# nubot-nudt/RDMNet

Hardware: AMD Instinct MI355X
Metric: scan-pairs/sec (whole node) (higher is better)
Workload: dtype f32

## Files before the change

### include/rdmnet_hip.h

```cpp
#ifndef RDMNET_HIP_H_
#define RDMNET_HIP_H_

#include <stddef.h>
#include <stdint.h>

#ifdef __cplusplus
extern "C" {
#endif

#define RDM_ABI_VERSION 2

int rdm_abi_version(void);
size_t rdm_abi_struct_size(int which);
const char* rdm_last_error(void);

int rdm_rehash_schedule(int64_t max_elems, int64_t* at_host, int64_t* buckets_host, int cap);

size_t rdm_grid_subsample_workspace_bytes(int64_t n_points, int batch);
int rdm_grid_subsample(const float* points, int64_t n_points, const int64_t* lengths, int batch,
                       float voxel_size, float* out_points, int64_t* out_lengths, void* ws,
                       size_t ws_bytes, void* stream);
int rdm_grid_subsample_form(const float* points, int64_t n_points, const int64_t* lengths, int batch, float voxel_size,
                            float* out_points, int64_t* out_lengths, void* ws, size_t ws_bytes, void* stream, int form);

// ... 47 lines not shown
                double* d2, double* totals_host, void* ws, size_t ws_bytes, void* stream);
int rdm_realign_error(const float* pts, int64_t n, int64_t ld, const double* gt_host, const double* est_host, double* mean_host,
                      void* ws, size_t ws_bytes, void* stream);

size_t rdm_information_workspace_bytes(int64_t n_q, int64_t n_s);
int rdm_information_matrix(const float* q, int64_t n_q, int64_t ld_q, const float* s, int64_t n_s, int64_t ld_s,
                           const double* q_transform_host, const double* s_transform_host, double cell, double radius,
                           double* out_host, int64_t* corr_out, int64_t capacity, void* ws, size_t ws_bytes, void* stream);

size_t rdm_gemm_workspace_bytes(int64_t m, int64_t n, int batches);
int rdm_gemm(const float* a, int64_t lda, int64_t stride_a, const float* b, int64_t ldb,
             int64_t stride_b, int trans_b, float* c, int64_t ldc, int64_t stride_c, int64_t m,
             int64_t n, int64_t k, int batches, const float* bias, const float* rowdiv, int act,
             void* ws, size_t ws_bytes, void* stream);
int rdm_gemm_last_plan(int* out4_host);

int rdm_kpconv_gather(const float* q_points, int64_t m, const float* s_points, int64_t n_s,
                      const float* s_feats, int64_t c, int64_t ldf, const uint8_t* s_positive,
                      const int64_t* idx, int64_t h, int64_t ldi, const int32_t* width,
                      const float* kernel_points, float sigma, float* wf, int64_t ldw, float* nn,
                      void* stream);
int rdm_kpconv_fused_enabled(void);
int rdm_kpconv_fused_supported(int64_t c_in, int64_t c_out);
int64_t rdm_kpconv_fused_partial_rows(int64_t m, int64_t c_in);
size_t rdm_kpconv_packed_floats(int64_t c_in, int64_t c_out);
int rdm_kpconv_pack_weights(const float* w_host, int64_t c_in, int64_t c_out, float* packed_host);
int rdm_kpconv_fused(const float* q_points, int64_t m, const float* s_points, int64_t n_s, const float* s_feats,
                     int64_t c, int64_t ldf, const uint8_t* s_positive, const int64_t* idx, int64_t h, int64_t ldi,
                     const int32_t* width, const float* kernel_points, float sigma, const float* w_packed,
                     const float* bias, int64_t c_out, float* out, int64_t ldo, double* gn_partial,
// ... 310 lines not shown
```

### rdmnet_amd/_lib.py

```python
import ctypes
import os

_HERE = os.path.dirname(os.path.abspath(__file__))
LIB_PATH = os.environ.get('RDM_LIB_PATH') or os.path.join(_HERE, 'librdmnet_hip.so')

c_void = ctypes.c_void_p
c_i64 = ctypes.c_int64
c_int = ctypes.c_int
c_f32 = ctypes.c_float
c_size = ctypes.c_size_t

ABI_VERSION = 2


class FineMatchingOptions(ctypes.Structure):
    _fields_ = [('topk', ctypes.c_int32), ('mutual', ctypes.c_int32), ('use_dustbin', ctypes.c_int32),
                ('use_global_score', ctypes.c_int32), ('confidence_threshold', ctypes.c_float),
                ('correspondence_limit', ctypes.c_int32)]

    @classmethod
    def of(cls, topk=1, mutual=False, use_dustbin=True, confidence_threshold=0.0, use_global_score=False,
           correspondence_limit=None):
        return cls(int(topk), int(bool(mutual)), int(bool(use_dustbin)), int(bool(use_global_score)), float(confidence_threshold),
                   0 if correspondence_limit is None else int(correspondence_limit))
# ... 28 lines not shown
    'rdm_grid_subsample': (c_int, [c_void, c_i64, c_void, c_int, c_f32, c_void, c_void, c_void, c_size,
                                   c_void]),
    'rdm_grid_subsample_form': (c_int, [c_void, c_i64, c_void, c_int, c_f32, c_void, c_void, c_void, c_size,
                                        c_void, c_int]),
    'rdm_radius_neighbors_workspace_bytes': (c_size, [c_i64, c_i64, c_int]),
    'rdm_radius_neighbors': (c_int, [c_void, c_i64, c_void, c_i64, c_void, c_void, c_int, c_f32, c_int,
                                     c_void, c_void, c_void, c_void, c_void, c_size, c_void]),
    'rdm_radius_grid_workspace_bytes': (c_size, [c_i64]),
    'rdm_radius_grid_build': (c_int, [c_void, c_i64, c_void, c_int, c_f32, c_void, c_size, c_void]),
    'rdm_radius_grid_query': (c_int, [c_void, c_size, c_i64, c_void, c_i64, c_void, c_int, c_f32, c_int, c_void, c_void,
                                      c_void, c_void, c_void, c_size, c_void]),
    'rdm_gemm_workspace_bytes': (c_size, [c_i64, c_i64, c_int]),
    'rdm_gemm': (c_int, [c_void, c_i64, c_i64, c_void, c_i64, c_i64, c_int, c_void, c_i64, c_i64, c_i64, c_i64,
                         c_i64, c_int, c_void, c_void, c_int, c_void, c_size, c_void]),
    'rdm_gemm_last_plan': (c_int, [c_void]),
    'rdm_kpconv_gather': (c_int, [c_void, c_i64, c_void, c_i64, c_void, c_i64, c_i64, c_void, c_void, c_i64,
                                  c_i64, c_void, c_void, c_f32, c_void, c_i64, c_void, c_void]),
    'rdm_kpconv_gather_ordered': (c_int, [c_void, c_i64, c_void, c_i64, c_void, c_i64, c_i64, c_void, c_void, c_i64,
                                          c_i64, c_void, c_void, c_f32, c_void, c_i64, c_void, c_void, c_void]),
    'rdm_kpconv_gather_form': (c_int, [c_void, c_i64, c_void, c_i64, c_void, c_i64, c_i64, c_void, c_void, c_i64,
                                       c_i64, c_void, c_void, c_f32, c_void, c_i64, c_void, c_void, c_int, c_void]),
    'rdm_kpconv_fused_enabled': (c_int, []),
    'rdm_kpconv_fused_supported': (c_int, [c_i64, c_i64]),
    'rdm_kpconv_fused_partial_rows': (c_i64, [c_i64, c_i64]),
    'rdm_kpconv_packed_floats': (c_size, [c_i64, c_i64]),
    'rdm_kpconv_pack_weights': (c_int, [c_void, c_i64, c_i64, c_void]),
    'rdm_kpconv_fused': (c_int, [c_void, c_i64, c_void, c_i64, c_void, c_i64, c_i64, c_void, c_void, c_i64, c_i64, c_void, c_void,
                                 c_f32, c_void, c_void, c_i64, c_void, c_i64, c_void, c_void, c_void]),
    'rdm_kpconv_fused_form': (c_int, [c_void, c_i64, c_void, c_i64, c_void, c_i64, c_i64, c_void, c_void, c_i64, c_i64, c_void, c_void,
                                      c_f32, c_void, c_void, c_i64, c_void, c_i64, c_void, c_void, c_int, c_void]),
# ... 195 lines not shown
```

### rdmnet_amd/csrc/engine.hip

```cpp
#include <algorithm>
#include <cmath>
#include <cstring>
#include <atomic>
#include <chrono>
#include <functional>
#include <map>
#include <memory>
#include <string>
#include <vector>

#include "../../include/rdmnet_hip.h"
#include <ctime>

#include "common.h"
#include "internal.h"
#include "lockstep.h"

namespace {

using namespace rdm;

struct Mat {
  float* p = nullptr;
  int64_t rows = 0, cols = 0, ld = 0;
// ... 944 lines not shown

extern "C" int rdm_engine_get_tensor(rdm_engine* e, const char* name, rdm_tensor_view* out) {
  RDM_REQUIRE(e && name && out, "rdm_engine_get_tensor: null pointer");
  auto it = e->taps.find(name);
  if (it == e->taps.end()) {
    set_error("rdm_engine_get_tensor: no tensor named %s (call rdm_engine_keep_taps first)", name);
    return RDM_ERR_ARG;
  }
  *out = it->second;
  return RDM_OK;
}

namespace {

struct PadGuard {
  explicit PadGuard(unsigned b) { rdm::gemm_set_lds_pad(b); }
  ~PadGuard() { rdm::gemm_set_lds_pad(0); }
};
struct CollateOnly {
  rdm_engine* e;
  bool keep_before;
  explicit CollateOnly(rdm_engine* eng) : e(eng), keep_before(eng->keep_taps) { e->keep_taps = e->collate_only = true; }
  ~CollateOnly() { e->collate_only = false; e->keep_taps = keep_before; }
};

int gs_multi_levels() {
  static const int n = [] { const char* v = ::rdm::dev_knob("RDM_GS_MULTI_LEVELS"); return v ? atoi(v) : 1; }();
  return n;
}

struct SearchQueue {
  std::vector<char> buf = std::vector<char>(radius_redo_queue_bytes());
// ... 76 lines not shown
static int grow_arena(rdm_engine* e, void* stream, const char* who) {
  RDM_HIP_CHECK(hipStreamSynchronize(static_cast<hipStream_t>(stream)));
  RDM_HIP_CHECK(hipFree(e->arena));
  e->arena = nullptr;
  e->arena_cap *= 2;
  const hipError_t err = hipMalloc(reinterpret_cast<void**>(&e->arena), e->arena_cap);
  if (err != hipSuccess) {
    e->arena_cap = 0;
    set_error("%s: growing the activation arena failed: %s", who, hipGetErrorString(err));
    return RDM_ERR_HIP;
  }
  return RDM_OK;
}
static int engine_run_growing(rdm_engine* e, const float* ref_points, int64_t n_ref, const float* src_points, int64_t n_src,
                              const rdm_data_dict* dd, rdm_engine_result* res, void* stream) {
  PadGuard pad_guard(e->pairs_in_flight >= 3 ? 20480u : 0u);
  for (;;) {
    e->arena_exhausted = false;
    const int rc = engine_run_once(e, ref_points, n_ref, src_points, n_src, dd, res, stream);
    if (!may_grow(e, rc)) return rc;
    ENG_CHECK(grow_arena(e, stream, "rdm_engine_run"));
  }
}

extern "C" int rdm_engine_run(rdm_engine* e, const float* ref_points, int64_t n_ref, const float* src_points,
                              int64_t n_src, rdm_engine_result* res, void* stream) {
  RDM_REQUIRE(e && ref_points && src_points && res, "rdm_engine_run: null pointer");
  RDM_REQUIRE(e->finalized, "rdm_engine_run: call rdm_engine_finalize first");
  RDM_REQUIRE(n_ref > 0 && n_src > 0, "rdm_engine_run: empty cloud");
  return engine_run_growing(e, ref_points, n_ref, src_points, n_src, nullptr, res, stream);
}
// ... 83 lines not shown
  for (;;) {
    e->arena_exhausted = false;
    const int rc = collate_batch_once(e, n_pairs, ref_points, n_ref, src_points, n_src, static_cast<hipStream_t>(stream));
    if (rc != RDM_OK) {
      e->batch.clear();
      e->arena_base = 0;
    }
    if (!may_grow(e, rc)) return rc;
    ENG_CHECK(grow_arena(e, stream, "rdm_engine_collate_batch"));
  }
}

extern "C" int rdm_engine_forward_batched(rdm_engine* e, int k, rdm_engine_result* res, void* stream) {
  RDM_REQUIRE(e && res, "rdm_engine_forward_batched: null pointer");
  RDM_REQUIRE(k >= 0 && k < static_cast<int>(e->batch.size()), "rdm_engine_forward_batched: no collated pair %d (rdm_engine_collate_batch first)", k);
  PadGuard pad_guard(e->pairs_in_flight >= 3 ? 20480u : 0u);
  e->arena_exhausted = false;
  return engine_run_once(e, nullptr, e->batch_n_ref[k], nullptr, e->batch_n_src[k], nullptr, res, stream, &e->batch[k]);
}

namespace {
int lockstep_wait(hipStream_t st, void* user) { return wait_idle(static_cast<rdm_engine*>(user), st); }

struct LockstepJob {
  const char* who;
  std::function<bool(int)> has_input;
  std::function<int(int)> check;
  std::function<int()> prepare;
  std::function<int(int)> pair;
  std::function<int(int)> rerun;
};

int lockstep_drive(const LockstepJob& job, rdm_engine* const* engines, rdm_engine_result* const* results, int n, void* stream) {
  const char* who = job.who;
  RDM_REQUIRE(n >= 1 && n <= kGroupMax, "%s: 1 .. %d pairs", who, kGroupMax);
  for (int k = 0; k < n; ++k) {
    RDM_REQUIRE(engines[k] && results[k] && job.has_input(k), "%s: pair %d is incomplete", who, k);
    RDM_REQUIRE(engines[k]->finalized, "%s: engine %d is not finalized", who, k);
    for (int j = 0; j < k; ++j) RDM_REQUIRE(engines[j] != engines[k], "%s: every pair needs an engine of its own", who);
    if (job.check) ENG_CHECK(job.check(k));
  }
  PadGuard pad_guard(0u);
  if (job.prepare) ENG_CHECK(job.prepare());
  struct Ctx {
    rdm_engine* const* engines;
    const LockstepJob* job;
  } ctx{engines, &job};
  auto run_pair = [](int k, void* user) -> int {
    const Ctx& c = *static_cast<const Ctx*>(user);
    c.engines[k]->arena_exhausted = false;
    return c.job->pair(k);
  };
  int rcs[kGroupMax] = {};
  const int wrc = lockstep_run(n, run_pair, &ctx, static_cast<hipStream_t>(stream), lockstep_wait, engines[0], rcs);
  if (wrc == -1) {
    set_error("%s: called from inside a lock-step group (a host thread runs one group at a time)", who);
    return RDM_ERR_ARG;
// ... 1096 lines not shown
```

### rdmnet_amd/csrc/gemm.hip

```cpp
#include "../../include/rdmnet_hip.h"
#include <cmath>
#include <cstdlib>

#include "common.h"
#include "internal.h"
#include "lockstep.h"

namespace {

using namespace rdm;

typedef float f32x16 __attribute__((ext_vector_type(16)));
typedef float f32x4_t __attribute__((ext_vector_type(4)));

struct GemmArgs {
  const float* A = nullptr;
  const float* B = nullptr;
  float* C = nullptr;
  const float* bias = nullptr;
  const float* rowdiv = nullptr;
  int M = 0, N = 0, K = 0;
  int lda = 0, ldb = 0, ldc = 0;
  long long sa = 0, sb = 0, sc = 0;
  int act = 0;
// ... 10 lines not shown
  unsigned long long* clk = nullptr;
#endif
};
#ifdef RDM_GEMM_TIMING
#define GEMM_STAMP(k) do { if (blockIdx.x == 0 && blockIdx.y == 0 && blockIdx.z == 0 && threadIdx.x == 0) g.clk[k] = __builtin_amdgcn_s_memtime(); } while (0)
#else
#define GEMM_STAMP(k) do { } while (0)
#endif

__device__ __forceinline__ float apply_act(float v, int act) {
  if (act == 1) return v > 0.f ? v : 0.f;
  if (act == 2) return v > 0.f ? v : 0.1f * v;
  return v;
}

template <int BM, int BN, int WM, int WN, int BK, bool TRANS_B, int PF, bool CAT = false>
__device__ __forceinline__ void gemm_kernel_body(const dim3 blockIdx, const dim3 gridDim, GemmArgs g) {
  (void)blockIdx; (void)gridDim;
  constexpr int TM = BM / WM, TN = BN / WN, FM = TM / 32, FN = TN / 32;
  static_assert(WM * WN == 4 && TM % 32 == 0 && TN % 32 == 0, "bad tile");
  constexpr int LDA_S = BM + 1, LDB_S = TRANS_B ? BN + 1 : BN + 4;
  constexpr int CR = BM < 64 ? BM : 64;
  constexpr int LDC_S = BN + 4;
  constexpr int TPR = BN / 4;
  constexpr int RPI = 256 / TPR;
  constexpr int kBytesAB = (2 * BK * LDA_S + 2 * BK * LDB_S) * 4, kBytesC = CR * LDC_S * 4, kBytesStat = RPI * BN * 2 * 8;
  constexpr int kBytes = kBytesAB > kBytesC ? (kBytesAB > kBytesStat ? kBytesAB : kBytesStat) : (kBytesC > kBytesStat ? kBytesC : kBytesStat);
  static_assert((2 * BK * LDA_S * 4) % 16 == 0 && CR % RPI == 0, "tile layout");
  __shared__ __attribute__((aligned(16))) char smem[kBytes];
  float (*As)[BK][LDA_S] = reinterpret_cast<float (*)[BK][LDA_S]>(smem);
  float (*Bs)[BK][LDB_S] = reinterpret_cast<float (*)[BK][LDB_S]>(smem + 2 * BK * LDA_S * 4);
  float (*Cs)[LDC_S] = reinterpret_cast<float (*)[LDC_S]>(smem);
  double (*stat_red)[1][2] = reinterpret_cast<double (*)[1][2]>(smem);

  const int tid = threadIdx.x, lane = tid & 63, wave = tid >> 6;
  const int wm = wave / WN, wn = wave % WN;
  int tile_x = blockIdx.x, tile_y = blockIdx.y;
  if (g.xcd_tiles) {
    const int nblk = gridDim.x * gridDim.y, lin = blockIdx.y * gridDim.x + blockIdx.x;
    const int q = nblk / 8, rr = nblk % 8, xcd = lin % 8, within = lin / 8;
    const int logical = (xcd < rr ? xcd * (q + 1) : rr * (q + 1) + (xcd - rr) * q) + within;
    tile_x = logical % gridDim.x;
    tile_y = logical / gridDim.x;
  }
  const int m0 = tile_y * BM, n0 = tile_x * BN;
  GEMM_STAMP(0);
  const int batch = blockIdx.z / g.splits, split = blockIdx.z % g.splits;
  const float* A = g.A + batch * g.sa;
  const float* B = g.B + batch * g.sb;

  const int ktiles = (g.K + BK - 1) / BK;
  const int per = (ktiles + g.splits - 1) / g.splits;
  const int kt0 = split * per, kt1 = min(ktiles, kt0 + per);

  constexpr int A_N4 = BM * BK / 4;
  constexpr int A_V = (A_N4 + 255) / 256;
  constexpr int KC4 = BK / 4;
  constexpr int B_N4 = BK * BN / 4;
  constexpr int B_V = (B_N4 + 255) / 256;
  static_assert(PF == 1 || PF == 2, "one or two register stages");
  float4 ra0[A_V], rb0[B_V], ra1[PF == 2 ? A_V : 1], rb1[PF == 2 ? B_V : 1];
  long long cat_row[CAT ? A_V : 1], cat_brow[CAT && TRANS_B ? B_V : 1];
  if constexpr (CAT && !TRANS_B) {
#pragma unroll
    for (int i = 0; i < A_V; ++i) {
      const int row = (tid + i * 256) / (BK / 4);
      const long long id = g.aidx[static_cast<long long>(min(m0 + row, g.M - 1)) * g.ldi];
      cat_row[i] = (id >= 0 && id < g.n_coarse) ? id : -1;
// ... 96 lines not shown
        Bs[buf][kc + 2][row] = v.z;
        Bs[buf][kc + 3][row] = v.w;
      }
    } else {
#pragma unroll
      for (int i = 0; i < B_V; ++i) {
        if (A_V + i < p0 || A_V + i >= p1) continue;
        const int idx = tid + i * 256;
        const int k = idx / (BN / 4), n4 = (idx % (BN / 4)) * 4;
        if (B_N4 % 256 != 0 && idx >= B_N4) continue;
        *reinterpret_cast<float4*>(&Bs[buf][k][n4]) = masked(rb[i], k0 + k < g.K && n0 + n4 < g.ldb);
      }
    }
  };

  const bool partial = g.splits > 1;
  const int c4 = (tid % TPR) * 4, rsub = tid / TPR;
  const int gcol = n0 + c4;
  float bv[4] = {0.f, 0.f, 0.f, 0.f};
  float rdv[BM / RPI];
  if (!partial && g.bias)
#pragma unroll
    for (int e = 0; e < 4; ++e) bv[e] = gcol + e < g.N ? g.bias[gcol + e] : 0.f;
#pragma unroll
  for (int q = 0; q < BM / RPI; ++q) rdv[q] = (!partial && g.rowdiv) ? g.rowdiv[min(m0 + q * RPI + rsub, g.M - 1)] : 1.f;

  f32x16 acc[FM][FN];
#pragma unroll
  for (int i = 0; i < FM; ++i)
#pragma unroll
    for (int j = 0; j < FN; ++j)
#pragma unroll
      for (int r = 0; r < 16; ++r) acc[i][j][r] = 0.f;

  const int lk = lane >> 5, li = lane & 31;
  constexpr int HK = BK / 2, HS = HK / 2;
  float af_lo[HS][FM], bf_lo[HS][FN], af_hi[HS][FM], bf_hi[HS][FN];
  auto read_kstep = [&](float (&af)[HS][FM], float (&bf)[HS][FN], int buf, int kbase, int s) {
#pragma unroll
    for (int i = 0; i < FM; ++i) af[s][i] = As[buf][kbase + 2 * s + lk][wm * TM + i * 32 + li];
#pragma unroll
    for (int j = 0; j < FN; ++j) bf[s][j] = Bs[buf][kbase + 2 * s + lk][wn * TN + j * 32 + li];
  };
  auto read_half = [&](float (&af)[HS][FM], float (&bf)[HS][FN], int buf, int kbase) {
#pragma unroll
    for (int s = 0; s < HS; ++s) read_kstep(af, bf, buf, kbase, s);
  };
  constexpr int NCH = HS * FM * FN, NP = A_V + B_V;
// ... 16 lines not shown
      acc[i][j] = __builtin_amdgcn_mfma_f32_32x32x2f32(af_hi[s][i], bf_hi[s][j], acc[i][j], 0, 0, 0);
      if (c % (FM * FN) == 0) read_kstep(af_lo, bf_lo, buf ^ 1, 0, s);
      __builtin_amdgcn_sched_barrier(0);
    }
  };
  if (kt0 < kt1) {
    load_tiles(ra0, rb0, kt0);
    if constexpr (PF == 2) load_tiles(ra1, rb1, kt0 + 1);
    store_tiles(ra0, rb0, 0, kt0);
  }
  lds_barrier();
  GEMM_STAMP(1);
  if (kt0 < kt1) {
    read_half(af_lo, bf_lo, 0, 0);
    if constexpr (PF == 1) {
      for (int kt = kt0; kt < kt1; ++kt) step(ra0, rb0, ra0, rb0, kt, (kt - kt0) & 1);
    } else {
      for (int kt = kt0; kt < kt1; kt += 2) {
        step(ra0, rb0, ra1, rb1, kt, 0);
        if (kt + 1 < kt1) step(ra1, rb1, ra0, rb0, kt + 1, 1);
      }
    }
  }

  GEMM_STAMP(2);
  const bool stats = g.stats != nullptr && !partial;
  const bool has_rd = !partial && g.rowdiv != nullptr;
  const int act = g.act;
  float* C = partial ? g.part + static_cast<long long>(blockIdx.z) * g.M * g.N : g.C + batch * g.sc;
  const int ldc = partial ? g.N : g.ldc;
  const bool vec_ok = (ldc & 3) == 0 && (reinterpret_cast<uintptr_t>(C) & 15) == 0;
  double cs[4] = {0.0, 0.0, 0.0, 0.0}, css[4] = {0.0, 0.0, 0.0, 0.0};
#pragma unroll
  for (int pass = 0; pass < BM / CR; ++pass) {
#pragma unroll
    for (int i = 0; i < FM; ++i) {
      const int rbase = wm * TM + i * 32 - pass * CR;
      if (rbase < 0 || rbase >= CR) continue;
#pragma unroll
      for (int j = 0; j < FN; ++j)
#pragma unroll
// ... 4 lines not shown
#pragma unroll
    for (int it = 0; it < CR / RPI; ++it) {
      const int lrow = it * RPI + rsub;
      const int row = m0 + pass * CR + lrow;
      if (row < g.M && gcol < g.N) {
        const float4 t = *reinterpret_cast<const float4*>(&Cs[lrow][c4]);
        float v[4] = {t.x, t.y, t.z, t.w};
        if (has_rd) {
          const float rd = rdv[pass * (CR / RPI) + it];
#pragma unroll
          for (int e = 0; e < 4; ++e) v[e] = v[e] / rd;
        }
        if (!partial) {
#pragma unroll
          for (int e = 0; e < 4; ++e) {
            const float u = v[e] + bv[e];
            const float neg = act == 2 ? 0.1f * u : 0.f;
            v[e] = (act != 0 && !(u > 0.f)) ? neg : u;
          }
        }
        float* dst = C + static_cast<long long>(row) * ldc + gcol;
        if (vec_ok && gcol + 3 < g.N) {
          *reinterpret_cast<float4*>(dst) = make_float4(v[0], v[1], v[2], v[3]);
        } else {
#pragma unroll
          for (int e = 0; e < 4; ++e)
            if (gcol + e < g.N) dst[e] = v[e];
        }
        if (stats) {
#pragma unroll
          for (int e = 0; e < 4; ++e) {
            cs[e] += v[e];
            css[e] += static_cast<double>(v[e]) * v[e];
          }
        }
      }
    }
    GEMM_STAMP(5);
    lds_barrier();
  }
  if (stats) {
#pragma unroll
    for (int e = 0; e < 4; ++e) {
      stat_red[rsub * BN + c4 + e][0][0] = cs[e];
      stat_red[rsub * BN + c4 + e][0][1] = css[e];
    }
    lds_barrier();
    for (int cl = tid; cl < BN; cl += 256) {
      const int col = n0 + cl;
      if (col >= g.N) continue;
      double a = 0.0, b = 0.0;
#pragma unroll
      for (int w = 0; w < RPI; ++w) {
        a += stat_red[w * BN + cl][0][0];
        b += stat_red[w * BN + cl][0][1];
      }
      g.stats[(static_cast<long long>(tile_y) * 2 + 0) * g.N + col] = a;
      g.stats[(static_cast<long long>(tile_y) * 2 + 1) * g.N + col] = b;
    }
  }
  GEMM_STAMP(3);
}
template <int BM, int BN, int WM, int WN, int BK, bool TRANS_B, int PF, bool CAT = false>
__global__ __launch_bounds__(256, (BM * BN <= 64 * 64 ? 4 : 1)) void gemm_kernel(GemmArgs g) { gemm_kernel_body<BM, BN, WM, WN, BK, TRANS_B, PF, CAT>(blockIdx, gridDim, g); }

__device__ __forceinline__ void gemm_small_body(const dim3 blockIdx, const GemmArgs& g, float (*red)[32][33]) {
  const int tid = threadIdx.x, lane = tid & 63, wave = tid >> 6;
  const int li = lane & 31, lk = lane >> 5;
  const int m0 = blockIdx.y * 32, n0 = blockIdx.x * 32;
  const int kq = g.K / 4;
  const int kbeg = wave * kq;
  const int row = min(m0 + li, g.M - 1);
  const int col = n0 + li;
  const bool col_ok = col < g.ldb;
  const float* arow = g.A + static_cast<long long>(row) * g.lda;
  f32x16 acc;
#pragma unroll
  for (int r = 0; r < 16; ++r) acc[r] = 0.f;
  for (int c = 0; c < kq; c += 32) {
// ... 298 lines not shown
    const int n = static_cast<int>(i % g.N);
    const int m = static_cast<int>((i / g.N) % g.M);
    const int b = static_cast<int>(i / (static_cast<long long>(g.M) * g.N));
    const float* p = g.part + (static_cast<long long>(b) * g.splits) * g.M * g.N +
                     static_cast<long long>(m) * g.N + n;
    float v = 0.f;
    for (int s = 0; s < g.splits; ++s) v += p[static_cast<long long>(s) * g.M * g.N];
    if (g.rowdiv) v = v / g.rowdiv[m];
    if (g.bias) v += g.bias[n];
    g.C[b * g.sc + static_cast<long long>(m) * g.ldc + n] = apply_act(v, g.act);
  }
}
__global__ void splitk_reduce_kernel(GemmArgs g, int batches) { splitk_reduce_kernel_body(blockIdx, gridDim, g, batches); }


constexpr int kStatRowsPerLane = 8;
inline int stat_rows_per_block(long long n) { return kStatRowsPerLane * (256 / static_cast<int>(n < 256 ? n : 256)); }
__device__ __forceinline__ void splitk_reduce_stats_kernel_body(const dim3 blockIdx, const dim3 gridDim, GemmArgs g, double* stats) {
  (void)blockIdx; (void)gridDim;
  __shared__ double red[2][256];
  const int cw = g.N < 256 ? g.N : 256;
  const int lanes = 256 / cw;
  const int r0 = blockIdx.x * (kStatRowsPerLane * lanes);
  const int r1 = min(g.M, r0 + kStatRowsPerLane * lanes);
  const int col_in = threadIdx.x % cw, rl = threadIdx.x / cw;
  const int col = blockIdx.y * 256 + col_in;
  double s = 0.0, ss = 0.0;
  if (rl < lanes && col < g.N) {
    const float bv = g.bias ? g.bias[col] : 0.f;
    const long long plane = static_cast<long long>(g.M) * g.N;
    float acc[kStatRowsPerLane];
// ... 27 lines not shown
  if (threadIdx.x < cw && col < g.N) {
    double a = 0.0, b = 0.0;
    for (int k = 0; k < lanes; ++k) {
      a += red[0][k * cw + threadIdx.x];
      b += red[1][k * cw + threadIdx.x];
    }
    stats[(static_cast<long long>(blockIdx.x) * 2 + 0) * g.N + col] = a;
    stats[(static_cast<long long>(blockIdx.x) * 2 + 1) * g.N + col] = b;
  }
}
__global__ __launch_bounds__(256) void splitk_reduce_stats_kernel(GemmArgs g, double* stats) { splitk_reduce_stats_kernel_body(blockIdx, gridDim, g, stats); }


thread_local unsigned g_lds_pad = 0;

template <int BM, int BN, int WM, int WN, int BK, int PF = 1>
void launch(const GemmArgs& g, int batches, bool trans_b, hipStream_t st) {
  dim3 grid(ceil_div(g.N, BN), ceil_div(g.M, BM), batches * g.splits);
  static const int pad_env = [] { const char* v = ::rdm::dev_knob("RDM_GEMM_LDS_PAD"); return v ? atoi(v) : -1; }();
  const unsigned pad = pad_env >= 0 ? static_cast<unsigned>(pad_env) : g_lds_pad;
  if constexpr (BM == 64 && BN == 64 && BK == 32 && PF == 2) {
    if (g.aidx && g.bidx) {
      ::rdm::launch<gemm_kernel_body<BM, BN, WM, WN, BK, true, PF, true>, gemm_kernel<BM, BN, WM, WN, BK, true, PF, true>, 256, (BM * BN <= 64 * 64 ? 4 : 1)>(grid, pad, st, g);
      return;
    }
    if (g.aidx) {
      ::rdm::launch<gemm_kernel_body<BM, BN, WM, WN, BK, false, PF, true>, gemm_kernel<BM, BN, WM, WN, BK, false, PF, true>, 256, (BM * BN <= 64 * 64 ? 4 : 1)>(grid, pad, st, g);
      return;
    }
  }
  if (trans_b)
    ::rdm::launch<gemm_kernel_body<BM, BN, WM, WN, BK, true, PF>, gemm_kernel<BM, BN, WM, WN, BK, true, PF>, 256, (BM * BN <= 64 * 64 ? 4 : 1)>(grid, pad, st, g);
  else
    ::rdm::launch<gemm_kernel_body<BM, BN, WM, WN, BK, false, PF>, gemm_kernel<BM, BN, WM, WN, BK, false, PF>, 256, (BM * BN <= 64 * 64 ? 4 : 1)>(grid, pad, st, g);
}

}

void rdm::gemm_set_lds_pad(unsigned bytes) { g_lds_pad = bytes; }

extern "C" size_t rdm_gemm_workspace_bytes(int64_t m, int64_t n, int batches) {
  const size_t by_shape = static_cast<size_t>(m) * static_cast<size_t>(n) * 16;
  const size_t by_tiles = static_cast<size_t>(1024) * 128 * 128;
  return align_up(std::min(by_shape, by_tiles) * sizeof(float) * static_cast<size_t>(batches > 0 ? batches : 1));
}

namespace {

thread_local int g_last_plan[4] = {0, 0, 0, 0};

enum Tile { T128, T64, T128x32 };

struct GemmPlan {
  bool small = false;
// ... 40 lines not shown
      double t = full * (c.fixed_us + k_per * per_k64(c.resident));
      if (rem) t += c.fixed_us + k_per * per_k64(static_cast<double>(ceil_div<long long>(rem, model_cus)));
      if (sp > 1) t += 3.0 + static_cast<double>(m) * n * sp * 8.0 / 1.5e6;
      if (t < best) {
        best = t;
        p.tile = c.tile;
        p.splits = sp;
      }
    }
  }
  if (g.aidx && g.bidx) p.splits = 1;
  set_tile_shape(p, k, g.aidx != nullptr);
  return p;
}

GemmPlan plan_gemm(const GemmArgs& g, int batches, bool trans_b, size_t ws_cap) {
  if (batches == 1 && !trans_b && !g.rowdiv && !g.stats && !g.aidx && small_kernel_ok(g.M, g.N, g.K)) {
    GemmPlan p;
    p.small = true;
    p.bm = p.bn = 32; p.bk = g.K / 4; p.splits = 4;
    return p;
  }
  return plan_tiled(g, batches, ws_cap);
}

#ifdef RDM_DEV_KNOBS

bool lab_tune_skips_small() {
  const char* tune = ::rdm::dev_knob("RDM_GEMM_TUNE");
  return tune && tune[0] != '0';
// ... 47 lines not shown

int launch_plan(const GemmPlan& p, GemmArgs g, int batches, bool trans_b, void* ws, int* stat_blocks, hipStream_t st) {
  const long long m = g.M, n = g.N;
  g_last_plan[0] = p.bm; g_last_plan[1] = p.bn; g_last_plan[2] = p.bk; g_last_plan[3] = p.splits;
  if (p.small) {
    if (stat_blocks) *stat_blocks = 0;
    RDM_DUP_LOOP("gemmsmall")
    ::rdm::launch<gemm_small_entry, gemm_small_kernel, 256>(dim3(ceil_div<long long>(n, 32), ceil_div<long long>(m, 32)), 0, st, g);
    return launch_status("gemm_small_kernel");
  }
  g.xcd_tiles = p.xcd_tiles;
  if (p.splits > 1) {
    g.splits = p.splits;
    g.part = static_cast<float*>(ws);
  }
  double* reduce_stats = nullptr;
  if (g.splits > 1) {
    if (batches == 1 && g.N % 4 == 0) reduce_stats = g.stats;
    g.stats = nullptr;
  }
  if (stat_blocks)
    *stat_blocks = g.stats ? static_cast<int>(ceil_div<long long>(m, p.bm))
                           : (reduce_stats ? static_cast<int>(ceil_div<long long>(m, stat_rows_per_block(n))) : 0);
  RDM_DUP_LOOP("gemm") {
#ifdef RDM_DEV_KNOBS
  if (p.exp_tile == 4) launch<128, 64, 2, 2, 32, 2>(g, batches, trans_b, st);
  else if (p.exp_tile == 5) launch<64, 128, 2, 2, 32, 2>(g, batches, trans_b, st);
  else if (p.exp_tile == 6) launch<128, 128, 2, 2, 32, 2>(g, batches, trans_b, st);
  else if (p.exp_tile == 7) launch<256, 64, 4, 1, 32, 2>(g, batches, trans_b, st);
  else
#endif
  switch (p.tile) {
    case T128: launch<128, 128, 2, 2, 16>(g, batches, trans_b, st); break;
    case T64:
      if (p.bk == 32) launch<64, 64, 2, 2, 32, 2>(g, batches, trans_b, st);
      else launch<64, 64, 2, 2, 16>(g, batches, trans_b, st);
      break;
    case T128x32:
      if (p.bk == 32) launch<128, 32, 4, 1, 32, 2>(g, batches, trans_b, st);
      else launch<128, 32, 4, 1, 16>(g, batches, trans_b, st);
      break;
  }
  }
  if (int e = launch_status("gemm_kernel")) return e;
  if (g.splits > 1 && reduce_stats) {
    RDM_DUP_LOOP("splitk")
    ::rdm::launch<splitk_reduce_stats_kernel_body, splitk_reduce_stats_kernel, 256>(dim3(ceil_div<long long>(m, stat_rows_per_block(n)), ceil_div<long long>(n, 256)), 0, st, g, reduce_stats);
    return launch_status("splitk_reduce_stats_kernel");
  }
  if (g.splits > 1) {
    const long long total = static_cast<long long>(batches) * m * n;
    const int blocks = static_cast<int>(std::min<long long>(ceil_div<long long>(total, 256), 2048));
    ::rdm::launch<splitk_reduce_kernel_body, splitk_reduce_kernel, 256>(dim3(blocks), 0, st, g, batches);
    return launch_status("splitk_reduce_kernel");
  }
  return RDM_OK;
}

int gemm_dispatch(const GemmArgs& g, int batches, bool trans_b, void* ws, size_t ws_bytes, int* stat_blocks, hipStream_t st) {
// ... 268 lines not shown
```

### rdmnet_amd/csrc/internal.h

```cpp
#pragma once
#include <cstddef>
#include <cstdint>

namespace rdm {

int gemm_with_stats(const float* a, int64_t lda, const float* b, int64_t ldb, float* c, int64_t ldc, int64_t m,
                    int64_t n, int64_t k, const float* bias, const float* rowdiv, void* ws, size_t ws_bytes,
                    double* gn_partial, int* gn_blocks, void* stream);

void gemm_set_lds_pad(unsigned bytes);
int gemm_concat_with_stats(const float* coarse, int64_t ld1, int64_t c1, int64_t n_coarse, const int64_t* idx, int64_t ldi,
                           const float* skip, int64_t ld2, int64_t c2, const float* b, int64_t ldb, float* c, int64_t ldc,
                           int64_t m, int64_t n, const float* bias, int act, void* ws, size_t ws_bytes, double* gn_partial,
                           int* gn_blocks, void* stream);

int gemm_pair(const float* a0, int64_t lda0, const float* b0, int64_t ldb0, float* c0, int64_t ldc0, int64_t m0, int64_t n0,
              int64_t k0, const float* bias0, const float* a1, int64_t lda1, const float* b1, int64_t ldb1, float* c1,
              int64_t ldc1, int64_t m1, int64_t n1, int64_t k1, const float* bias1, void* ws, size_t ws_bytes, void* stream);

inline int64_t gemm_stats_max_blocks(int64_t m) { return (m + 7) / 8 + 1; }

int grid_subsample_mode(const float* points, int64_t n_points, const int64_t* lengths, int batch, float voxel_size,
                        float* out_points, int64_t* out_lengths, void* ws, size_t ws_bytes, void* stream, int mode);

int group_norm_finish(const double* partial, int nblk, const float* x, int64_t n, int64_t c, int64_t ldx, int groups,
// ... 41 lines not shown
```

### rdmnet_amd/ops.py

```python
import ctypes

import torch

from . import _lib, config

ACT_NONE, ACT_RELU, ACT_LEAKY = 0, 1, 2


def pad4(n):
    return (int(n) + 3) // 4 * 4


class Scratch:

    def __init__(self, device):
        self.device = device
        self.buf = torch.empty(1 << 24, dtype=torch.uint8, device=device)

    def get(self, nbytes):
        if self.buf.numel() < nbytes:
            self.buf = torch.empty(int(nbytes * 1.25) + 256, dtype=torch.uint8, device=self.device)
        return self.buf


# ... 19 lines not shown


def gemm(a, b, k, n, *, trans_b=False, bias=None, rowdiv=None, act=ACT_NONE, out=None):
    L = _lib.lib()
    m = a.shape[0]
    if a.stride(-1) != 1 or b.stride(-1) != 1:
        raise ValueError('gemm operands must be row-major (unit column stride)')
    if out is None:
        out = feat_empty(m, n, a.device)
    ws_bytes = L.rdm_gemm_workspace_bytes(m, n, 1)
    ws = scratch(a.device, ws_bytes)
    _lib.check(L.rdm_gemm(a.data_ptr(), _ld(a), 0, b.data_ptr(), _ld(b), 0, int(trans_b), out.data_ptr(), _ld(out),
                          0, m, n, k, 1, _lib.ptr(bias), _lib.ptr(rowdiv), act, ws.data_ptr(), ws.numel(),
                          _lib.stream_ptr()), 'rdm_gemm')
    return out


def gemm_batched(a, b, k, *, trans_b=True, out=None, rowdiv=None):
    L = _lib.lib()
    B, m, n = a.shape[0], a.shape[1], b.shape[1]
    if out is None:
        out = torch.empty((B, m, n), dtype=torch.float32, device=a.device)
    _lib.check(L.rdm_gemm(a.data_ptr(), a.stride(1), a.stride(0), b.data_ptr(), b.stride(1), b.stride(0),
                          int(trans_b), out.data_ptr(), out.stride(1), out.stride(0), m, n, k, B, 0, _lib.ptr(rowdiv), ACT_NONE, 0, 0,
                          _lib.stream_ptr()), 'rdm_gemm(batched)')
    return out


def patch_scores(ref_feats, ref_idx, src_feats, src_idx, rowdiv=None):
    L = _lib.lib()
# ... 969 lines not shown
```

### rdmnet_amd/pipeline.py

```python
import os
import threading
import time

import numpy as np
import torch

from .engine import Engine

DEFAULT_PAIRS_IN_FLIGHT = 4
DEFAULT_STAGGER_MS = 1.5
DEFAULT_COLLATE_BATCH = 1
DEFAULT_LOCKSTEP = 4


def _quota_cpus():
    try:
        quota, period = open('/sys/fs/cgroup/cpu.max').read().split()[:2]
        return float('inf') if quota == 'max' else float(quota) / float(period)
    except (OSError, ValueError):
        try:
            q = float(open('/sys/fs/cgroup/cpu/cpu.cfs_quota_us').read())
            per = float(open('/sys/fs/cgroup/cpu/cpu.cfs_period_us').read())
            return q / per if q > 0 else float('inf')
        except (OSError, ValueError):
# ... 105 lines not shown

    def __init__(self, eng, res, ms):
        self.transform = eng.transform()
        self.ref_corr_points, self.src_corr_points, self.corr_scores = eng.host_corr()
        self.n_correspondences = int(res.n_correspondences)
        self.n_ref_nodes, self.n_src_nodes = int(res.n_ref_nodes), int(res.n_src_nodes)
        self.n_node_correspondences = int(res.n_node_correspondences)
        self.level_sizes = [int(x) for x in res.level_sizes]
        self.ms = ms


class PairPipeline:

    def __init__(self, cfg, state, device=None, pairs_in_flight=DEFAULT_PAIRS_IN_FLIGHT, wait_us=None,
                 stagger_ms=DEFAULT_STAGGER_MS, keep_taps=False, local_world=None, engines=None, streams=None,
                 collate_batch=DEFAULT_COLLATE_BATCH, lockstep=None, arena_bytes=None):
        self._gpu = torch.cuda.is_available()
        if not self._gpu and engines is None:
            raise RuntimeError('rdmnet_amd.pipeline needs a GPU (no CPU fallback)')
        self.device = (torch.device('cuda', torch.cuda.current_device()) if device is None else torch.device(device)) if self._gpu else None
        self.n = max(1, int(pairs_in_flight))
        self.collate_batch = max(1, int(collate_batch))
        if lockstep is None:
            lockstep = DEFAULT_LOCKSTEP if (engines is None and self.n >= 2) else 1
        self.lockstep = max(1, min(8, int(lockstep)))
        self.keep_taps = bool(keep_taps)
        self.stagger_s = max(0.0, float(stagger_ms)) * 1e-3
        local_world = int(os.environ.get('LOCAL_WORLD_SIZE', '1')) if local_world is None else local_world
        self.wait_us = choose_wait_us(self.n, local_world) if wait_us is None or wait_us < 0 else int(wait_us)
        if streams is not None:
            self.streams = list(streams)
        else:
# ... 76 lines not shown
                while len(got) < want:
                    try:
                        slot, job = next(it)
                    except StopIteration:
                        state['exhausted'] = True
                        break
                    state['drawn'] = slot + 1
                    got.append((slot, job))
                return got or None

        def worker(k):
            stream = self.streams[k]
            import contextlib
            torch.set_num_threads(1)
            try:
                with (torch.cuda.device(self.device) if self._gpu else contextlib.nullcontext()):
                    ctx = torch.cuda.stream(stream) if stream is not None else None
                    if ctx is not None:
                        ctx.__enter__()
                    try:
                        if stagger and k > 0 and self.stagger_s > 0:
                            time.sleep(k * self.stagger_s)
                        while True:
                            t0 = time.perf_counter()
                            with cv:
                                while state['drawn'] - state['next_out'] >= window and not state['stop']:
                                    cv.wait(timeout=0.05)
                            t1 = time.perf_counter()
                            got = draw()
                            t2 = time.perf_counter()
# ... 102 lines not shown
```

Before: 597.0.

## Add serial split-K GEMM form that accumulates in-kernel when pairs run concurrently

Adds a SERIAL variant of the tiled GEMM kernel. One block walks all K tiles and folds the per-split partial accumulators in registers, instead of writing partial planes and launching a separate split-K reduce kernel. Group-norm statistics are computed in the epilogue through LDS. The variant is chosen automatically when several pairs are in flight, since concurrent streams already fill the GPU. This removes the partial-plane traffic and the reduce launch, but gives up the K-parallelism that split-K provided and adds register pressure from the second accumulator set.

Result: slower. 585.4 (-1.9%).

```diff
diff --git a/include/rdmnet_hip.h b/include/rdmnet_hip.h
--- a/include/rdmnet_hip.h
+++ b/include/rdmnet_hip.h
@@ -85,6 +85,7 @@
              int64_t n, int64_t k, int batches, const float* bias, const float* rowdiv, int act,
              void* ws, size_t ws_bytes, void* stream);
 int rdm_gemm_last_plan(int* out4_host);
+int rdm_gemm_set_split_mode(int mode);
 
 int rdm_kpconv_gather(const float* q_points, int64_t m, const float* s_points, int64_t n_s,
                       const float* s_feats, int64_t c, int64_t ldf, const uint8_t* s_positive,
diff --git a/rdmnet_amd/_lib.py b/rdmnet_amd/_lib.py
--- a/rdmnet_amd/_lib.py
+++ b/rdmnet_amd/_lib.py
@@ -66,6 +66,7 @@
     'rdm_gemm': (c_int, [c_void, c_i64, c_i64, c_void, c_i64, c_i64, c_int, c_void, c_i64, c_i64, c_i64, c_i64,
                          c_i64, c_int, c_void, c_void, c_int, c_void, c_size, c_void]),
     'rdm_gemm_last_plan': (c_int, [c_void]),
+    'rdm_gemm_set_split_mode': (c_int, [c_int]),
     'rdm_kpconv_gather': (c_int, [c_void, c_i64, c_void, c_i64, c_void, c_i64, c_i64, c_void, c_void, c_i64,
                                   c_i64, c_void, c_void, c_f32, c_void, c_i64, c_void, c_void]),
     'rdm_kpconv_gather_ordered': (c_int, [c_void, c_i64, c_void, c_i64, c_void, c_i64, c_i64, c_void, c_void, c_i64,
diff --git a/rdmnet_amd/csrc/engine.hip b/rdmnet_amd/csrc/engine.hip
--- a/rdmnet_amd/csrc/engine.hip
+++ b/rdmnet_amd/csrc/engine.hip
@@ -982,8 +982,8 @@
 namespace {
 
 struct PadGuard {
-  explicit PadGuard(unsigned b) { rdm::gemm_set_lds_pad(b); }
-  ~PadGuard() { rdm::gemm_set_lds_pad(0); }
+  PadGuard(unsigned b, int pairs) { rdm::gemm_set_lds_pad(b); rdm::gemm_set_pairs_in_flight(pairs); }
+  ~PadGuard() { rdm::gemm_set_lds_pad(0); rdm::gemm_set_pairs_in_flight(1); }
 };
 struct CollateOnly {
   rdm_engine* e;
@@ -1090,7 +1090,7 @@
 }
 static int engine_run_growing(rdm_engine* e, const float* ref_points, int64_t n_ref, const float* src_points, int64_t n_src,
                               const rdm_data_dict* dd, rdm_engine_result* res, void* stream) {
-  PadGuard pad_guard(e->pairs_in_flight >= 3 ? 20480u : 0u);
+  PadGuard pad_guard(e->pairs_in_flight >= 3 ? 20480u : 0u, e->pairs_in_flight);
   for (;;) {
     e->arena_exhausted = false;
     const int rc = engine_run_once(e, ref_points, n_ref, src_points, n_src, dd, res, stream);
@@ -1204,7 +1204,7 @@
 extern "C" int rdm_engine_forward_batched(rdm_engine* e, int k, rdm_engine_result* res, void* stream) {
   RDM_REQUIRE(e && res, "rdm_engine_forward_batched: null pointer");
   RDM_REQUIRE(k >= 0 && k < static_cast<int>(e->batch.size()), "rdm_engine_forward_batched: no collated pair %d (rdm_engine_collate_batch first)", k);
-  PadGuard pad_guard(e->pairs_in_flight >= 3 ? 20480u : 0u);
+  PadGuard pad_guard(e->pairs_in_flight >= 3 ? 20480u : 0u, e->pairs_in_flight);
   e->arena_exhausted = false;
   return engine_run_once(e, nullptr, e->batch_n_ref[k], nullptr, e->batch_n_src[k], nullptr, res, stream, &e->batch[k]);
 }
@@ -1230,7 +1230,7 @@
     for (int j = 0; j < k; ++j) RDM_REQUIRE(engines[j] != engines[k], "%s: every pair needs an engine of its own", who);
     if (job.check) ENG_CHECK(job.check(k));
   }
-  PadGuard pad_guard(0u);
+  PadGuard pad_guard(0u, std::max(n, engines[0]->pairs_in_flight));
   if (job.prepare) ENG_CHECK(job.prepare());
   struct Ctx {
     rdm_engine* const* engines;
diff --git a/rdmnet_amd/csrc/gemm.hip b/rdmnet_amd/csrc/gemm.hip
--- a/rdmnet_amd/csrc/gemm.hip
+++ b/rdmnet_amd/csrc/gemm.hip
@@ -48,7 +48,9 @@
   return v;
 }
 
-template <int BM, int BN, int WM, int WN, int BK, bool TRANS_B, int PF, bool CAT = false>
+constexpr int kStatRowsPerLane = 8;
+
+template <int BM, int BN, int WM, int WN, int BK, bool TRANS_B, int PF, bool CAT = false, bool SERIAL = false>
 __device__ __forceinline__ void gemm_kernel_body(const dim3 blockIdx, const dim3 gridDim, GemmArgs g) {
   (void)blockIdx; (void)gridDim;
   constexpr int TM = BM / WM, TN = BN / WN, FM = TM / 32, FN = TN / 32;
@@ -79,13 +81,13 @@
   }
   const int m0 = tile_y * BM, n0 = tile_x * BN;
   GEMM_STAMP(0);
-  const int batch = blockIdx.z / g.splits, split = blockIdx.z % g.splits;
+  const int batch = SERIAL ? blockIdx.z : blockIdx.z / g.splits, split = SERIAL ? 0 : blockIdx.z % g.splits;
   const float* A = g.A + batch * g.sa;
   const float* B = g.B + batch * g.sb;
 
   const int ktiles = (g.K + BK - 1) / BK;
   const int per = (ktiles + g.splits - 1) / g.splits;
-  const int kt0 = split * per, kt1 = min(ktiles, kt0 + per);
+  const int kt0 = split * per, kt1 = SERIAL ? ktiles : min(ktiles, kt0 + per);
 
   constexpr int A_N4 = BM * BK / 4;
   constexpr int A_V = (A_N4 + 255) / 256;
@@ -212,16 +214,19 @@
     }
   };
 
-  const bool partial = g.splits > 1;
+  const bool partial = !SERIAL && g.splits > 1;
   const int c4 = (tid % TPR) * 4, rsub = tid / TPR;
   const int gcol = n0 + c4;
   float bv[4] = {0.f, 0.f, 0.f, 0.f};
   float rdv[BM / RPI];
-  if (!partial && g.bias)
-#pragma unroll
-    for (int e = 0; e < 4; ++e) bv[e] = gcol + e < g.N ? g.bias[gcol + e] : 0.f;
-#pragma unroll
-  for (int q = 0; q < BM / RPI; ++q) rdv[q] = (!partial && g.rowdiv) ? g.rowdiv[min(m0 + q * RPI + rsub, g.M - 1)] : 1.f;
+  auto load_epilogue_operands = [&]() {
+    if (!partial && g.bias)
+#pragma unroll
+      for (int e = 0; e < 4; ++e) bv[e] = gcol + e < g.N ? g.bias[gcol + e] : 0.f;
+#pragma unroll
+    for (int q = 0; q < BM / RPI; ++q) rdv[q] = (!partial && g.rowdiv) ? g.rowdiv[min(m0 + q * RPI + rsub, g.M - 1)] : 1.f;
+  };
+  if constexpr (!SERIAL || BM * BN > 64 * 64) load_epilogue_operands();
 
   f32x16 acc[FM][FN];
 #pragma unroll
@@ -230,6 +235,37 @@
     for (int j = 0; j < FN; ++j)
 #pragma unroll
       for (int r = 0; r < 16; ++r) acc[i][j][r] = 0.f;
+  f32x16 tot[SERIAL ? FM : 1][SERIAL ? FN : 1];
+  if constexpr (SERIAL) {
+#pragma unroll
+    for (int i = 0; i < FM; ++i)
+#pragma unroll
+      for (int j = 0; j < FN; ++j)
+#pragma unroll
+        for (int r = 0; r < 16; ++r) tot[i][j][r] = 0.f;
+  }
+  auto fold = [&]() {
+    if constexpr (SERIAL) {
+#pragma unroll
+      for (int i = 0; i < FM; ++i)
+#pragma unroll
+        for (int j = 0; j < FN; ++j)
+#pragma unroll
+          for (int r = 0; r < 16; ++r) {
+            tot[i][j][r] += acc[i][j][r];
+            acc[i][j][r] = 0.f;
+          }
+    }
+  };
+  int range_left = per;
+  auto tile_done = [&]() {
+    if constexpr (SERIAL) {
+      if (--range_left == 0) {
+        fold();
+        range_left = per;
+      }
+    }
+  };
 
   const int lk = lane >> 5, li = lane & 31;
   constexpr int HK = BK / 2, HS = HK / 2;
@@ -276,17 +312,34 @@
   if (kt0 < kt1) {
     read_half(af_lo, bf_lo, 0, 0);
     if constexpr (PF == 1) {
-      for (int kt = kt0; kt < kt1; ++kt) step(ra0, rb0, ra0, rb0, kt, (kt - kt0) & 1);
+      for (int kt = kt0; kt < kt1; ++kt) {
+        step(ra0, rb0, ra0, rb0, kt, (kt - kt0) & 1);
+        tile_done();
+      }
     } else {
       for (int kt = kt0; kt < kt1; kt += 2) {
         step(ra0, rb0, ra1, rb1, kt, 0);
-        if (kt + 1 < kt1) step(ra1, rb1, ra0, rb0, kt + 1, 1);
+        tile_done();
+        if (kt + 1 < kt1) {
+          step(ra1, rb1, ra0, rb0, kt + 1, 1);
+          tile_done();
+        }
       }
     }
   }
+  if constexpr (SERIAL && BM * BN <= 64 * 64) load_epilogue_operands();
+  if constexpr (SERIAL) {
+    for (int s = ktiles / per; s < g.splits; ++s) fold();
+#pragma unroll
+    for (int i = 0; i < FM; ++i)
+#pragma unroll
+      for (int j = 0; j < FN; ++j) acc[i][j] = tot[i][j];
+  }
 
   GEMM_STAMP(2);
-  const bool stats = g.stats != nullptr && !partial;
+  const bool stats = !SERIAL && g.stats != nullptr && !partial;
+  const bool rstats = SERIAL && g.stats != nullptr;
+  const bool add_bias = !SERIAL || g.bias != nullptr || rstats;
   const bool has_rd = !partial && g.rowdiv != nullptr;
   const int act = g.act;
   float* C = partial ? g.part + static_cast<long long>(blockIdx.z) * g.M * g.N : g.C + batch * g.sc;
@@ -321,7 +374,7 @@
         if (!partial) {
 #pragma unroll
           for (int e = 0; e < 4; ++e) {
-            const float u = v[e] + bv[e];
+            const float u = add_bias ? v[e] + bv[e] : v[e];
             const float neg = act == 2 ? 0.1f * u : 0.f;
             v[e] = (act != 0 && !(u > 0.f)) ? neg : u;
           }
@@ -334,6 +387,8 @@
           for (int e = 0; e < 4; ++e)
             if (gcol + e < g.N) dst[e] = v[e];
         }
+        if constexpr (SERIAL)
+          if (rstats) *reinterpret_cast<float4*>(&Cs[lrow][c4]) = make_float4(v[0], v[1], v[2], v[3]);
         if (stats) {
 #pragma unroll
           for (int e = 0; e < 4; ++e) {
@@ -345,6 +400,34 @@
     }
     GEMM_STAMP(5);
     lds_barrier();
+    if constexpr (SERIAL) {
+      if (rstats) {
+        const int cw = g.N < 256 ? g.N : 256, lanes = 256 / cw, rb = kStatRowsPerLane * lanes;
+        for (int w = tid; w < (CR / rb) * BN; w += 256) {
+          const int cl = w % BN, lr0 = (w / BN) * rb;
+          const int col = n0 + cl, r0 = m0 + pass * CR + lr0;
+          if (col >= g.N || r0 >= g.M) continue;
+          const int r1 = min(g.M, r0 + rb);
+          double a = 0.0, b = 0.0;
+          for (int rl = 0; rl < lanes; ++rl) {
+            double s = 0.0, ss = 0.0;
+#pragma unroll
+            for (int u = 0; u < kStatRowsPerLane; ++u) {
+              const int r = r0 + rl + u * lanes;
+              if (r >= r1) break;
+              const double d = Cs[lr0 + rl + u * lanes][cl];
+              s += d;
+              ss += d * d;
+            }
+            a += s;
+            b += ss;
+          }
+          g.stats[(static_cast<long long>(r0 / rb) * 2 + 0) * g.N + col] = a;
+          g.stats[(static_cast<long long>(r0 / rb) * 2 + 1) * g.N + col] = b;
+        }
+        lds_barrier();
+      }
+    }
   }
   if (stats) {
 #pragma unroll
@@ -368,8 +451,8 @@
   }
   GEMM_STAMP(3);
 }
-template <int BM, int BN, int WM, int WN, int BK, bool TRANS_B, int PF, bool CAT = false>
-__global__ __launch_bounds__(256, (BM * BN <= 64 * 64 ? 4 : 1)) void gemm_kernel(GemmArgs g) { gemm_kernel_body<BM, BN, WM, WN, BK, TRANS_B, PF, CAT>(blockIdx, gridDim, g); }
+template <int BM, int BN, int WM, int WN, int BK, bool TRANS_B, int PF, bool CAT = false, bool SERIAL = false>
+__global__ __launch_bounds__(256, (BM * BN <= 64 * 64 ? 4 : 1)) void gemm_kernel(GemmArgs g) { gemm_kernel_body<BM, BN, WM, WN, BK, TRANS_B, PF, CAT, SERIAL>(blockIdx, gridDim, g); }
 
 __device__ __forceinline__ void gemm_small_body(const dim3 blockIdx, const GemmArgs& g, float (*red)[32][33]) {
   const int tid = threadIdx.x, lane = tid & 63, wave = tid >> 6;
@@ -698,7 +781,6 @@
 __global__ void splitk_reduce_kernel(GemmArgs g, int batches) { splitk_reduce_kernel_body(blockIdx, gridDim, g, batches); }
 
 
-constexpr int kStatRowsPerLane = 8;
 inline int stat_rows_per_block(long long n) { return kStatRowsPerLane * (256 / static_cast<int>(n < 256 ? n : 256)); }
 __device__ __forceinline__ void splitk_reduce_stats_kernel_body(const dim3 blockIdx, const dim3 gridDim, GemmArgs g, double* stats) {
   (void)blockIdx; (void)gridDim;
@@ -756,30 +838,46 @@
 
 thread_local unsigned g_lds_pad = 0;
 
-template <int BM, int BN, int WM, int WN, int BK, int PF = 1>
+template <int BM, int BN, int WM, int WN, int BK, int PF = 1, bool SERIAL = false>
 void launch(const GemmArgs& g, int batches, bool trans_b, hipStream_t st) {
-  dim3 grid(ceil_div(g.N, BN), ceil_div(g.M, BM), batches * g.splits);
+  dim3 grid(ceil_div(g.N, BN), ceil_div(g.M, BM), SERIAL ? batches : batches * g.splits);
   static const int pad_env = [] { const char* v = ::rdm::dev_knob("RDM_GEMM_LDS_PAD"); return v ? atoi(v) : -1; }();
   const unsigned pad = pad_env >= 0 ? static_cast<unsigned>(pad_env) : g_lds_pad;
   if constexpr (BM == 64 && BN == 64 && BK == 32 && PF == 2) {
+    if constexpr (!SERIAL) {
     if (g.aidx && g.bidx) {
       ::rdm::launch<gemm_kernel_body<BM, BN, WM, WN, BK, true, PF, true>, gemm_kernel<BM, BN, WM, WN, BK, true, PF, true>, 256, (BM * BN <= 64 * 64 ? 4 : 1)>(grid, pad, st, g);
       return;
     }
+    }
     if (g.aidx) {
-      ::rdm::launch<gemm_kernel_body<BM, BN, WM, WN, BK, false, PF, true>, gemm_kernel<BM, BN, WM, WN, BK, false, PF, true>, 256, (BM * BN <= 64 * 64 ? 4 : 1)>(grid, pad, st, g);
+      ::rdm::launch<gemm_kernel_body<BM, BN, WM, WN, BK, false, PF, true, SERIAL>, gemm_kernel<BM, BN, WM, WN, BK, false, PF, true, SERIAL>, 256, (BM * BN <= 64 * 64 ? 4 : 1)>(grid, pad, st, g);
       return;
     }
   }
   if (trans_b)
-    ::rdm::launch<gemm_kernel_body<BM, BN, WM, WN, BK, true, PF>, gemm_kernel<BM, BN, WM, WN, BK, true, PF>, 256, (BM * BN <= 64 * 64 ? 4 : 1)>(grid, pad, st, g);
+    ::rdm::launch<gemm_kernel_body<BM, BN, WM, WN, BK, true, PF, false, SERIAL>, gemm_kernel<BM, BN, WM, WN, BK, true, PF, false, SERIAL>, 256, (BM * BN <= 64 * 64 ? 4 : 1)>(grid, pad, st, g);
   else
-    ::rdm::launch<gemm_kernel_body<BM, BN, WM, WN, BK, false, PF>, gemm_kernel<BM, BN, WM, WN, BK, false, PF>, 256, (BM * BN <= 64 * 64 ? 4 : 1)>(grid, pad, st, g);
+    ::rdm::launch<gemm_kernel_body<BM, BN, WM, WN, BK, false, PF, false, SERIAL>, gemm_kernel<BM, BN, WM, WN, BK, false, PF, false, SERIAL>, 256, (BM * BN <= 64 * 64 ? 4 : 1)>(grid, pad, st, g);
 }
 
 }
 
 void rdm::gemm_set_lds_pad(unsigned bytes) { g_lds_pad = bytes; }
+
+namespace {
+thread_local int g_split_mode = 0;
+thread_local int g_pairs_in_flight = 1;
+}
+
+void rdm::gemm_set_pairs_in_flight(int n) { g_pairs_in_flight = n > 1 ? n : 1; }
+
+extern "C" int rdm_gemm_set_split_mode(int mode) {
+  using namespace rdm;
+  RDM_REQUIRE(mode >= 0 && mode <= 2, "rdm_gemm_set_split_mode: mode %d (0 = automatic, 1 = partial planes, 2 = serial)", mode);
+  g_split_mode = mode;
+  return RDM_OK;
+}
 
 extern "C" size_t rdm_gemm_workspace_bytes(int64_t m, int64_t n, int batches) {
   const size_t by_shape = static_cast<size_t>(m) * static_cast<size_t>(n) * 16;
@@ -850,6 +948,17 @@
   return p;
 }
 
+bool serial_form_ok(const GemmPlan& p, const GemmArgs& g, int batches) {
+  if (p.small || p.splits <= 1 || p.exp_tile) return false;
+  if (p.bk != (p.tile == T128 ? 16 : 32)) return false;
+  if (g.stats && batches == 1 && g.N % 4 == 0) {
+    const int rb = stat_rows_per_block(g.N);
+    if (rb > 64 || 64 % rb != 0) return false;
+  }
+  return true;
+}
+bool serial_form_auto(const GemmPlan& p, int pairs_in_flight) { return p.splits > 1 && pairs_in_flight >= 2; }
+
 GemmPlan plan_gemm(const GemmArgs& g, int batches, bool trans_b, size_t ws_cap) {
   if (batches == 1 && !trans_b && !g.rowdiv && !g.stats && !g.aidx && small_kernel_ok(g.M, g.N, g.K)) {
     GemmPlan p;
@@ -927,13 +1036,21 @@
     g.splits = p.splits;
     g.part = static_cast<float*>(ws);
   }
+  bool serial = false;
+  if (g.splits > 1 && serial_form_ok(p, g, batches)) {
+    serial = g_split_mode == 2 || (g_split_mode == 0 && serial_form_auto(p, g_pairs_in_flight));
+#ifdef RDM_DEV_KNOBS
+    static const int serial_env = [] { const char* v = ::rdm::dev_knob("RDM_GEMM_SERIAL_SPLIT"); return v ? atoi(v) : -1; }();
+    if (serial_env >= 0) serial = serial_env != 0;
+#endif
+  }
   double* reduce_stats = nullptr;
   if (g.splits > 1) {
     if (batches == 1 && g.N % 4 == 0) reduce_stats = g.stats;
-    g.stats = nullptr;
+    g.stats = serial ? reduce_stats : nullptr;
   }
   if (stat_blocks)
-    *stat_blocks = g.stats ? static_cast<int>(ceil_div<long long>(m, p.bm))
+    *stat_blocks = (g.stats && !serial) ? static_cast<int>(ceil_div<long long>(m, p.bm))
                            : (reduce_stats ? static_cast<int>(ceil_div<long long>(m, stat_rows_per_block(n))) : 0);
   RDM_DUP_LOOP("gemm") {
 #ifdef RDM_DEV_KNOBS
@@ -943,6 +1060,11 @@
   else if (p.exp_tile == 7) launch<256, 64, 4, 1, 32, 2>(g, batches, trans_b, st);
   else
 #endif
+  if (serial) {
+    if (p.tile == T128) launch<128, 128, 2, 2, 16, 1, true>(g, batches, trans_b, st);
+    else if (p.tile == T64) launch<64, 64, 2, 2, 32, 2, true>(g, batches, trans_b, st);
+    else launch<128, 32, 4, 1, 32, 2, true>(g, batches, trans_b, st);
+  } else
   switch (p.tile) {
     case T128: launch<128, 128, 2, 2, 16>(g, batches, trans_b, st); break;
     case T64:
@@ -956,6 +1078,7 @@
   }
   }
   if (int e = launch_status("gemm_kernel")) return e;
+  if (serial) return RDM_OK;
   if (g.splits > 1 && reduce_stats) {
     RDM_DUP_LOOP("splitk")
     ::rdm::launch<splitk_reduce_stats_kernel_body, splitk_reduce_stats_kernel, 256>(dim3(ceil_div<long long>(m, stat_rows_per_block(n)), ceil_div<long long>(n, 256)), 0, st, g, reduce_stats);
diff --git a/rdmnet_amd/csrc/internal.h b/rdmnet_amd/csrc/internal.h
--- a/rdmnet_amd/csrc/internal.h
+++ b/rdmnet_amd/csrc/internal.h
@@ -9,6 +9,7 @@
                     double* gn_partial, int* gn_blocks, void* stream);
 
 void gemm_set_lds_pad(unsigned bytes);
+void gemm_set_pairs_in_flight(int n);
 int gemm_concat_with_stats(const float* coarse, int64_t ld1, int64_t c1, int64_t n_coarse, const int64_t* idx, int64_t ldi,
                            const float* skip, int64_t ld2, int64_t c2, const float* b, int64_t ldb, float* c, int64_t ldc,
                            int64_t m, int64_t n, const float* bias, int act, void* ws, size_t ws_bytes, double* gn_partial,
diff --git a/rdmnet_amd/ops.py b/rdmnet_amd/ops.py
--- a/rdmnet_amd/ops.py
+++ b/rdmnet_amd/ops.py
@@ -57,6 +57,17 @@
                           0, m, n, k, 1, _lib.ptr(bias), _lib.ptr(rowdiv), act, ws.data_ptr(), ws.numel(),
                           _lib.stream_ptr()), 'rdm_gemm')
     return out
+
+
+def gemm_set_split_mode(mode):
+    _lib.check(_lib.lib().rdm_gemm_set_split_mode(int(mode)), 'rdm_gemm_set_split_mode')
+
+
+def gemm_last_plan():
+    import ctypes
+    out = (ctypes.c_int * 4)()
+    _lib.check(_lib.lib().rdm_gemm_last_plan(ctypes.addressof(out)), 'rdm_gemm_last_plan')
+    return tuple(out)
 
 
 def gemm_batched(a, b, k, *, trans_b=True, out=None, rowdiv=None):
diff --git a/rdmnet_amd/pipeline.py b/rdmnet_amd/pipeline.py
--- a/rdmnet_amd/pipeline.py
+++ b/rdmnet_amd/pipeline.py
@@ -143,8 +143,9 @@
 
     def __init__(self, cfg, state, device=None, pairs_in_flight=DEFAULT_PAIRS_IN_FLIGHT, wait_us=None,
                  stagger_ms=DEFAULT_STAGGER_MS, keep_taps=False, local_world=None, engines=None, streams=None,
-                 collate_batch=DEFAULT_COLLATE_BATCH, lockstep=None, arena_bytes=None):
+                 collate_batch=DEFAULT_COLLATE_BATCH, lockstep=None, arena_bytes=None, split_mode=None):
         self._gpu = torch.cuda.is_available()
+        self.split_mode = None if split_mode is None else int(split_mode)
         if not self._gpu and engines is None:
             raise RuntimeError('rdmnet_amd.pipeline needs a GPU (no CPU fallback)')
         self.device = (torch.device('cuda', torch.cuda.current_device()) if device is None else torch.device(device)) if self._gpu else None
@@ -251,6 +252,9 @@
             import contextlib
             torch.set_num_threads(1)
             try:
+                if self.split_mode is not None:
+                    from . import ops
+                    ops.gemm_set_split_mode(self.split_mode)
                 with (torch.cuda.device(self.device) if self._gpu else contextlib.nullcontext()):
                     ctx = torch.cuda.stream(stream) if stream is not None else None
                     if ctx is not None:
```
